# Hitenze/Preconditioned_Additive_Gaussian_Processes_with_Fourier_Acceleration

Hardware: AMD Instinct MI355X
Metric: kernel matvecs/sec + PCG wall-time to 1e-6, n=1e6 d=32 additive, 1/2/4/8 GPU (higher is better)
Workload: dtype f64; 1 GPU; additive NFFT matvec, n=1000000, d=32, 32 x 1-D windows, Gaussian f=1 l=1 mu=0.01 (BASELINE configs[2]); n=1000000, d=32, nwindows=32, parallelism=single

## Files before the change

preconditioned_additive_gaussian_processes_with_fourier_acceleration_amd/csrc/internal.h:

```cpp
#pragma once

#include <hip/hip_runtime.h>

#include <cstdint>
#include <cstdio>
#include <memory>
#include <utility>
#include <string>
#include <vector>

#include "../../include/nfft4gp_amd.h"

namespace nfft4gp_amd {

constexpr int kNos = 64;
constexpr int kBand = 32;
constexpr int kM = 4;
constexpr int kTaps = 2 * kM + 2;
constexpr int kDeg = 7;
constexpr int kNC = kDeg + 1;
constexpr int kR = 16;
constexpr int kWave = 64;
constexpr int kPad = 32;
constexpr int kMaxBlock = 4096 - kPad;
// ... 77 lines not shown
struct AdditivePlan;
int build_layout_dev(const uint32_t* d_qc, int n, int nw, int B, int CG, AdditivePlan& P, hipStream_t s, int rec = 5);

struct DevLayout {
   uint16_t* meta = nullptr;
   uint32_t* lo = nullptr;
   uint32_t* q = nullptr;
   int* tile_off = nullptr;
   int* cmax = nullptr;
   long long ntiles = 0;
   size_t bytes = 0;
};

constexpr int kMdMaxDim = 5;
constexpr int kMdTiledMaxDim = 3;
struct MdComp {
   int d = 0;
   int hicount = 1;
   long long u_off = 0;
};
struct MdPlan {
   bool on = false;
   bool gfix_per_window = false;
   int maxd = 1;
   long long G = 0;
   long long Cmax = 0;
   long long M = 0;
   std::vector<MdComp> comps;
   MdComp* d_comps = nullptr;
   int* d_u = nullptr;
   double* d_psi = nullptr;
   double* d_grid = nullptr;
   double2* d_F[2] = {nullptr, nullptr};
   double2* d_Mo[2] = {nullptr, nullptr};
   double2* d_B[4] = {nullptr, nullptr, nullptr, nullptr};
   double* d_h[2] = {nullptr, nullptr};
   double* d_bh = nullptr;
   double* d_bhd = nullptr;
   double* d_dot_part = nullptr;
   unsigned int* d_dot_ticket = nullptr;
   int* d_perm = nullptr;
   int4* d_items = nullptr;
   int nitems = 0;
   bool lines = false;
   double* d_part = nullptr;
   unsigned long long* d_gfix = nullptr;
   unsigned long long* d_xmax = nullptr;
   double psi_max = 0.0;
};

struct AdditivePlan {
   int n_global = 0, row_begin = 0, row_end = 0, n = 0;
   int nw = 0, dw = 0, skip_last = 0;
   std::vector<int> comp_dims;
   int d = 0;
   std::vector<int> comp_feature;
   bool points_ready = false;
   std::vector<double> comp_scale;
   std::vector<double> comp_centre;
   std::vector<double> comp_sigma;
   int kernel = 0;
   double f = 1.0, l = 1.0, mu = 0.0;
   double weight = 1.0;
   double diag = 1.0;
   int B = kMaxBlock, CG = 3, ngroups = 0, nblocks = 0;
   int rec = 5;
   int spread_variant = -1;
   int spread_fold = 1;
   bool det = false;
   double* d_hb = nullptr;
   int nparts = 0;
   DevLayout dl;
   double* d_part = nullptr;
   double* d_w = nullptr;
   double* d_wd = nullptr;
   double* d_H = nullptr;
   double* d_Hd = nullptr;
   double* d_C = nullptr;
   double* d_dot_part = nullptr;
   unsigned int* d_dot_ticket = nullptr;
   double* d_part2 = nullptr;
   double* d_gsum = nullptr;
   int fused_grid = -1;
   bool cells33 = false;
   double* d_hsum = nullptr;
   int hsum_par = 0;
   double* d_H2 = nullptr;
   double* d_xs = nullptr;
   double* d_ys = nullptr;
   MdPlan md;
   bool timing = false;
   hipEvent_t* kev = nullptr;
   double ms[3] = {0, 0, 0};
   long long cnt[3] = {0, 0, 0};
};

int upload_tap_coeffs();
int launch_spread(const AdditivePlan& P, const double* d_x, double* d_part, hipStream_t stream);
int launch_grid(const AdditivePlan& P, const double* d_part, int nparts, int grad, hipStream_t stream);
int launch_spread_grid(AdditivePlan& P, const double* d_x, int grad, hipStream_t stream);
int launch_grid_from_sum(const AdditivePlan& P, const double* d_gridsum, int grad, hipStream_t stream);
constexpr int kPeerInline = 8;
struct PeerArgs {
   char* const* bufs = nullptr;
   char* inl[kPeerInline] = {};
   char* own = nullptr;
   int world = 0;
   unsigned int epoch = 0;
   unsigned int* err = nullptr;
   long long slot_doubles = 0;
   long long spin = 0;
};
int launch_reduce_parts(const AdditivePlan& P, const double* d_part, double* d_gridsum, hipStream_t stream,
                        const PeerArgs* A = nullptr);
int launch_shard_finish_split(const AdditivePlan& P, const double* d_gridsum, double alpha, const double* d_x,
                              double beta, double* d_y, int S, hipStream_t stream, const PeerArgs* A = nullptr,
                              const double* d_part = nullptr);
int launch_peer_grid(const AdditivePlan& P, const PeerArgs& A, const double* d_part, hipStream_t stream);
int launch_peer_sum(const AdditivePlan& P, const PeerArgs& A, double* d_grid, hipStream_t stream);
int launch_interp(const AdditivePlan& P, int grad, double alpha, const double* d_x, double beta, double* d_y,
                  hipStream_t stream, double* d_dot = nullptr);
int launch_interp_blocks(const AdditivePlan& P, double alpha, const double* d_x, double beta, double* d_y, int b0,
                         int b1, hipStream_t stream);
int launch_matvec2(AdditivePlan& P, double alpha, const double* x0, const double* x1, double beta, double* y0,
                   double* y1, hipStream_t stream);
int pick_spread_variant(const AdditivePlan& P);
bool grid_atomic(const AdditivePlan& P);
int pick_interp_threads(const AdditivePlan& P);
bool pick_interp_hl(const AdditivePlan& P);
int pick_hl_slots(const AdditivePlan& P);
int pick_interp2_threads();
bool pick_fused_grid(const AdditivePlan& P);
int launch_matvec_fused(AdditivePlan& P, double alpha, const double* d_x, double beta, double* d_y, hipStream_t stream,
                        double* d_dot = nullptr);
int additive_matvec_multi(void* str, int nv, double alpha, const double* const* X, double beta, double* const* Y);
int additive_matvec_dot(void* str, const double* d_x, double* d_y, double* d_dot);
AdditivePlan* additive_plan_of(void* str);
bool additive_fused_dot_ok(void* str);

struct NysDev {
   int n = 0, k = 0;
   double eta = 0.0;
   double* U = nullptr;
   float* Uf = nullptr;
   double* s = nullptr;
   double* w = nullptr;
   double* part = nullptr;
   int nblk = 0;
   double setup_ms[4] = {0.0, 0.0, 0.0, 0.0};
   std::vector<double> hs;
   bool grad = false;
   double f2 = 0.0;
   double *Kall = nullptr, *dU = nullptr, *G = nullptr, *Gt = nullptr, *GdKG = nullptr, *D = nullptr;
   double *vk = nullptr, *vn = nullptr;
};
void nys_free(NysDev* N);
constexpr int kNysRows = 2048;
int nys_alloc_scratch(NysDev* N);
int gemm_f64(bool transA, int M, int N, int K, const double* A, long long lda, const double* B, long long ldb,
             double* C, long long ldc, hipStream_t s);
int sym_eig_host(const std::vector<double>& A, int n, std::vector<double>& w, std::vector<double>& V);
int chol_inverse_host(std::vector<double>& A, int k);
int lu_solve_host(std::vector<double>& A, int n, std::vector<double>& B, int nrhs, double* logabsdet = nullptr,
                  int* sign = nullptr, std::vector<int>* piv_out = nullptr);
void lu_subst_host(const std::vector<double>& A, int n, const std::vector<int>& piv, std::vector<double>& B, int nrhs);
int lu_solve_dev(double* A, int n, double* B, int nrhs, hipStream_t s, double* logabsdet = nullptr,
// ... 161 lines not shown
```

preconditioned_additive_gaussian_processes_with_fourier_acceleration_amd/csrc/nfft_api.cpp:

```cpp
#include <dlfcn.h>
#include <hip/hip_runtime.h>

#include <array>
#include <algorithm>
#include <atomic>
#include <chrono>
#include <thread>
#include <cmath>
#include <cstdio>
#include <cstdlib>
#include <cstring>
#include <mutex>
#include <vector>

#include "internal.h"
#include "reduce.hpp"

using namespace nfft4gp_amd;

namespace nfft4gp_amd {

namespace {
std::recursive_mutex g_rand_mu;
int g_rand_depth = 0;
// ... 416 lines not shown
   if (!dy) {
      yd = P.d_ys;
      if (beta != 0.0) NFFT4GP_HIP_CHECK(hipMemcpyAsync(yd, y, sizeof(double) * ny, hipMemcpyHostToDevice, s));
   }
   if (plan_apply_dev(E, grad, alpha, xd, beta, yd)) return -1;
   if (!dy) NFFT4GP_HIP_CHECK(hipMemcpyAsync(y, yd, sizeof(double) * ny, hipMemcpyDeviceToHost, s));
   NFFT4GP_HIP_CHECK(hipStreamSynchronize(s));
   return 0;
}

PlanExt* additive_plan(void* str)
{
   if (!str) return nullptr;
   return (PlanExt*)((nfft4gp_kernel*)str)->_external;
}


int omp_threads_in_process()
{
   using fn_t = int (*)();
   static fn_t f = (fn_t)dlsym(RTLD_DEFAULT, "omp_get_max_threads");
   return f ? std::max(1, f()) : 1;
}

nfft4gp_kernel* kernel_struct_create(int max_n, int omp = 0)
{
   nfft4gp_kernel* k = (nfft4gp_kernel*)calloc(1, sizeof(nfft4gp_kernel));
   k->_max_n = max_n;
   k->_omp = omp;
   k->_ldwork = (size_t)max_n * (size_t)(omp ? omp_threads_in_process() : 1);
   k->_dwork = (double*)malloc(sizeof(double) * std::max<size_t>(1, k->_ldwork));
   return k;
}

int setup_common(void* str, int kernel, int n, int ldim, double** Kp, double** dKp)
{
   if (Kp == NULL || dKp == NULL) {
      printf("Error: NFFT kernel requires Kp and dKp to be not NULL.\n");
      return -1;
   }
   nfft4gp_kernel* kd = (nfft4gp_kernel*)str;
   PlanExt* E = additive_plan(str);
   if (!E) return -1;
   (void)n;
   (void)ldim;
   if (plan_setup(E->P, kd->_buffer, kernel, kd->_params[0], kd->_params[1], kd->_noise_level)) return -1;
   *Kp = (double*)str;
   *dKp = (double*)str;
   return 0;
}

int default_block(int n)
{
   if (n >= 200 * kMaxBlock) return kMaxBlock;
   if (n >= 40 * 2032) return 2032;
   return 1024;
}

void env_layout(AdditivePlan& P)
{
   P.B = default_block(P.n);
   {
      const int nw = std::max(P.nw, 1), nblocks = std::max(1, (P.n + P.B - 1) / P.B);
      auto pick = [&](int cgmax) {
         const int ngroups = (nw + cgmax - 1) / cgmax;
         P.CG = (nw + ngroups - 1) / ngroups;
         return ngroups;
      };
      if ((long long)pick(4) * nblocks < 384) pick(3);
   }
   if (const char* e = getenv("NFFT4GP_AMD_BLOCK")) {
      const int v = atoi(e);
      if (v >= 256) P.B = std::min(v, kMaxBlock) & ~15;
   }
   if (const char* e = getenv("NFFT4GP_AMD_CG")) {
      const int v = atoi(e);
      if (v >= 1 && v <= 64) P.CG = v;
   }
   if (const char* e = getenv("NFFT4GP_AMD_SPREAD_VARIANT")) P.spread_variant = atoi(e);
   if (const char* e = getenv("NFFT4GP_AMD_SPREAD_FOLD")) P.spread_fold = atoi(e) != 0;
   if (const char* e = getenv("NFFT4GP_AMD_DET")) P.det = atoi(e) != 0;
   if (const char* e = getenv("NFFT4GP_AMD_PRECISION")) P.rec = atoi(e) == 32 ? 4 : 5;
   if (const char* e = getenv("NFFT4GP_AMD_FUSED_GRID")) P.fused_grid = atoi(e) != 0;
}

void* additive_create(double* data, int n_global, int ldim, int d, int* windows, int nwindows, int dwindows, int rb,
                      int re)
{
   nfft4gp_kernel* kd = kernel_struct_create(3 * n_global);
   kd->_iparams[0] = nwindows;
   kd->_iparams[1] = dwindows;
   int skip_window = 1;
   kd->_iparams[2] = 0;
   while (skip_window < dwindows && windows[nwindows * dwindows - skip_window] < 0) {
      skip_window++;
      kd->_iparams[2]++;
   }
   kd->_ibufferp = (int**)malloc(sizeof(int*));
   kd->_ibufferp[0] = windows;
   kd->_buffer = (double*)malloc(sizeof(double) * (size_t)n_global * nwindows * dwindows);
   kd->_own_buffer = 1;
   PlanExt* E = new PlanExt();
   AdditivePlan& P = E->P;
   P.n_global = n_global;
   P.row_begin = rb;
   P.row_end = re;
   P.n = re - rb;
   P.nw = nwindows;
   P.dw = dwindows;
   P.d = d;
   P.skip_last = kd->_iparams[2];
   P.weight = 1.0 / (double)nwindows;
   env_layout(P);
   double* dst = kd->_buffer;
   const int* fw = windows;
   for (int i = 0; i < nwindows; i++) {
      int actual = 0;
      for (int j = 0; j < dwindows; j++) {
         if (fw[0] >= 0) {
            memcpy(dst, data + (size_t)fw[0] * ldim, sizeof(double) * n_global);
            if (actual == 0) P.comp_feature.push_back(fw[0]);
            fw++;
            dst += n_global;
            actual++;
         }
      }
      if (actual == 0) P.comp_feature.push_back(-1);
      P.comp_dims.push_back(actual);
   }
   kd->_external = E;
   return kd;
}

}

namespace nfft4gp_amd {
bool additive_fused_dot_ok(void* str)
{
   PlanExt* E = additive_plan(str);
   if (!E || !E->P.points_ready) return false;
   const AdditivePlan& P = E->P;
   if (P.row_begin != 0 || P.row_end != P.n_global) return false;
   return P.md.on || P.nblocks <= kRedMaxBlocks;
}

int additive_matvec_dot(void* str, const double* d_x, double* d_y, double* d_dot)
{
   PlanExt* E = additive_plan(str);
   if (!E || !E->P.points_ready) return -1;
   AdditivePlan& P = E->P;
   hipStream_t s = current_stream();
   if (P.md.on) {
      if (md_spread(P, d_x, P.md.d_grid, s) || md_grid(P, P.md.d_grid, 0, s)) return -1;
      return md_interp(P, 0, 1.0, d_x, 0.0, d_y, s, d_dot);
   }
   if (use_fused(P, s)) return launch_matvec_fused(P, 1.0, d_x, 0.0, d_y, s, d_dot);
   if (launch_spread_grid(P, d_x, 0, s)) return -1;
   return launch_interp(P, 0, 1.0, d_x, 0.0, d_y, s, d_dot);
}
}

namespace nfft4gp_amd {
int additive_matvec_multi(void* str, int nv, double alpha, const double* const* X, double beta, double* const* Y)
{
   PlanExt* E = additive_plan(str);
   if (!E || !E->P.points_ready) return -1;
// ... 662 lines not shown
```

preconditioned_additive_gaussian_processes_with_fourier_acceleration_amd/csrc/nfft_kernels.hip:

```cpp
#include <hip/hip_ext.h>
#include <hip/hip_runtime.h>

#include <algorithm>
#include <cmath>
#include <cstdio>
#include <vector>

#include "internal.h"
#include "reduce.hpp"

namespace nfft4gp_amd {

constexpr int kGridThreads = 1024;
constexpr int kMomStride = kNC + 1;
constexpr int kMomWin = kNC * kNos + 4;
template <int MOMT>
__host__ __device__ constexpr int mom_doubles_per_window()
{
   return MOMT ? kMomWin : kNos * kMomStride;
}
template <int MOMT>
__device__ __forceinline__ int mom_index(int cl, int cell, int d)
{
   return MOMT ? cl * kMomWin + d * kNos + cell : (cl * kNos + cell) * kMomStride + d;
// ... 96 lines not shown
   const int per = (nloc + nwaves - 1) / nwaves;
   const uint32_t* hw = reinterpret_cast<const uint32_t*>(s_alpha);
   uint32_t m = 0;
   for (int e = wave * per + lane; e < min(nloc, (wave + 1) * per); e += 64) m = max(m, hw[2 * e + 1] & 0x7FFFFFFFu);
   for (int off = 32; off > 0; off >>= 1) m = max(m, (uint32_t)__shfl_xor((int)m, off, 64));
   if (lane == 0) {
      s_red[wave] = m;
      __hip_atomic_fetch_add(s_red + nwaves, 1u, __ATOMIC_RELEASE, __HIP_MEMORY_SCOPE_WORKGROUP);
   }
}
template <int THREADS>
__device__ __forceinline__ uint32_t det_max_wait(uint32_t* s_red)
{
   constexpr int nwaves = THREADS / 64;
   while (__hip_atomic_load(s_red + nwaves, __ATOMIC_ACQUIRE, __HIP_MEMORY_SCOPE_WORKGROUP) < (uint32_t)nwaves)
      __builtin_amdgcn_s_sleep(1);
   uint32_t m = 0;
#pragma unroll
   for (int w = 0; w < nwaves; w++) m = max(m, s_red[w]);
   return (uint32_t)__builtin_amdgcn_readfirstlane((int)m) >> 20;
}

__device__ __forceinline__ uint32_t det_interp_exp(const double* __restrict__ hb, int nw)
{
   double Y = 0.0;
   for (int c = 0; c < nw; c++) Y += hb[c];
   const uint32_t bY = ((uint32_t)__double2hiint(Y) >> 20) & 0x7FFu;
   return min(bY + 2u, 2046u);
}

template <int REC>
__device__ __forceinline__ int tile_at(TileRegs& cur, const uint16_t* __restrict__ meta,
                                       const uint32_t* __restrict__ lo, const uint32_t* __restrict__ qarr, int t, int t1)
{
   if (t < t1) load_tile<REC>(cur, meta, lo, qarr, t, threadIdx.x & 63);
   return t;
}

__device__ __forceinline__ void gather_h(double (&h)[kNC], const double* __restrict__ H, uint32_t mt)
{
   const double2* src = reinterpret_cast<const double2*>(H + (size_t)mt * kNC);
#pragma unroll
   for (int d = 0; d < kNC; d += 2) {
      const double2 v = src[d / 2];
      h[d] = v.x;
      h[d + 1] = v.y;
   }
}
__device__ __forceinline__ void gather_h_lds(double (&h)[kNC], const double* row, int stride)
{
#pragma unroll
   for (int d = 0; d < kNC; d++) h[d] = row[d * stride];
}

template <int REC, bool DET>
__device__ __forceinline__ void interp_run(const TileRegs& cur, const double (&h)[kNC], double C)
{
#pragma unroll
   for (int r = 0; r < kR; r++) {
      const uint32_t off = slot_off<REC>(cur, r);
      const double u = q_to_s(cur.qq[r]);
      double v = h[kNC - 1];
#pragma unroll
      for (int d = kNC - 2; d >= 0; d--) v = fma(v, u, h[d]);
      lds_add(off, DET ? det_round(v, C) : v);
   }
}

constexpr int kEpMax = 8;

template <int THREADS>
__device__ __forceinline__ void ep_prefetch(double (&xe)[kEpMax], double (&ye)[kEpMax], const double* __restrict__ x,
                                            const double* __restrict__ y, int base, int nloc, double beta)
{
   static_assert(kMaxBlock <= kEpMax * THREADS, "a block's epilogue values fit the threads' registers");
#pragma unroll
   for (int k = 0; k < kEpMax; k++) {
      const int j = threadIdx.x + k * THREADS;
      xe[k] = (j < nloc) ? x[(size_t)base + j] : 0.0;
      ye[k] = (beta != 0.0 && j < nloc) ? y[(size_t)base + j] : 0.0;
   }
}

template <int THREADS, bool DOT>
__device__ __forceinline__ double ep_plain(const double (&xe)[kEpMax], const double (&ye)[kEpMax], const double* s_y,
                                           double* __restrict__ y, int base, int nloc, double alpha, double beta,
                                           double f, double mu)
{
   const double ff = f * f;
   double dacc = 0.0;
#pragma unroll
   for (int k = 0; k < kEpMax; k++) {
      const int j = threadIdx.x + k * THREADS;
      if (j >= nloc) break;
      const double v = ff * (s_y[j] + mu * xe[k]);
      const double yo = (beta == 0.0) ? alpha * v : fma(beta, ye[k], alpha * v);
      y[(size_t)base + j] = yo;
      if (DOT) dacc = fma(yo, xe[k], dacc);
   }
   return dacc;
}

template <int THREADS>
__device__ __forceinline__ void ep_dot_finish(double dacc, double* s_scr, double* __restrict__ dot_part,
                                              unsigned int* __restrict__ dot_ticket, double* __restrict__ dot_out)
{
   dacc = block_sum0_s<THREADS>(dacc, s_scr);
   double tot;
   if (grid_total_s<THREADS>(dacc, dot_part, dot_ticket, &tot, reinterpret_cast<int*>(s_scr + 2 * (THREADS / 64)),
                             s_scr + THREADS / 64) &&
       threadIdx.x == 0)
      *dot_out = tot;
}

constexpr bool kFoldMfmaOk = kNC == 8 && kTaps <= 12 && kNos == 64;
template <int REC>
__device__ __forceinline__ void fold_tap_operand(double (&a)[2], int lane)
{
   const int i = lane & 15, k = lane >> 4;
   const double* ct = REC == 4 ? c_taps_u : c_taps;
#pragma unroll
   for (int ks = 0; ks < 2; ks++) a[ks] = i < kTaps ? ct[i * kNC + 4 * ks + k] : 0.0;
}
__device__ __forceinline__ double fold_window_mfma(const double (&a)[2], double* mrow, double* grow89, int lane)
{
   typedef double f64x4 __attribute__((ext_vector_type(4)));
   const int i = lane & 15, k = lane >> 4;
   double bm[2][4];
#pragma unroll
   for (int ks = 0; ks < 2; ks++)
#pragma unroll
      for (int cb = 0; cb < 4; cb++) bm[ks][cb] = mrow[(4 * ks + k) * kNos + 16 * cb + i];
#pragma unroll
   for (int cb = 0; cb < 4; cb++) {
      f64x4 acc = {0.0, 0.0, 0.0, 0.0};
      acc = __builtin_amdgcn_mfma_f64_16x16x4f64(a[0], bm[0][cb], acc, 0, 0, 0);
      acc = __builtin_amdgcn_mfma_f64_16x16x4f64(a[1], bm[1][cb], acc, 0, 0, 0);
      mrow[k * kNos + 16 * cb + i] = acc[0];
      mrow[(4 + k) * kNos + 16 * cb + i] = acc[1];
      if (k < kTaps - 8) grow89[k * kNos + 16 * cb + i] = acc[2];
   }
   __builtin_amdgcn_fence(__ATOMIC_RELEASE, "wavefront");
   __builtin_amdgcn_wave_barrier();
   __builtin_amdgcn_fence(__ATOMIC_ACQUIRE, "wavefront");
   double v = 0.0;
#pragma unroll
   for (int tp = 0; tp < kTaps; tp++) {
      const int cell = (lane + kM - tp) & (kNos - 1);
      v += tp < 8 ? mrow[tp * kNos + cell] : grow89[(tp - 8) * kNos + cell];
   }
   return v;
}

constexpr int kFgCells = 33;
constexpr int kFgSpan = kFgCells + kTaps - 1;
constexpr int kFgSpan0 = (kNos - 16 - kM) & (kNos - 1);

template <int THREADS, bool TIMELINE = false, int MOMT = 1, bool DET = false, int REC = 5, bool PIPE = false>
__global__ __launch_bounds__(THREADS, 6) void k_spread(const uint16_t* __restrict__ meta,
                                                      const uint32_t* __restrict__ lo,
                                                      const uint32_t* __restrict__ qarr,
                                                      const int* __restrict__ tile_off, const int* __restrict__ cmax,
                                                      const double* __restrict__ x, int n, int B, int nblocks,
                                                      int ngroups, int CG, int nw, double* __restrict__ part,
                                                      double* __restrict__ gsum, int fold)
{
   extern __shared__ __attribute__((aligned(16))) double smem[];
   const int Bp = B + kPad;
   double* s_alpha = smem;
   double* s_mom = smem + Bp;
   uint32_t* s_red = reinterpret_cast<uint32_t*>(s_mom + CG * mom_doubles_per_window<MOMT>());

   const int xcd = blockIdx.x & 7;
   const int rest = blockIdx.x >> 3;
   const int g = rest % ngroups;
   const int b = (rest / ngroups) * 8 + xcd;
   if (b >= nblocks) return;
   if (TIMELINE) stamp(0);

   const int tid = threadIdx.x;
// ... 563 lines not shown
   }
}

template <int THREADS, bool DET = false, int REC = 5>
__global__ __launch_bounds__(THREADS) void k_interp_hl(const uint16_t* __restrict__ meta, const uint32_t* __restrict__ lo,
                                                       const uint32_t* __restrict__ qarr, const int* __restrict__ tile_off,
                                                       const double* __restrict__ H, const double* __restrict__ x,
                                                       double* __restrict__ y, int n, int B, int ngroups, int CG, int nw,
                                                       double alpha, double beta, double f, double mu,
                                                       const double* __restrict__ hb, int ns)
{
   extern __shared__ __attribute__((aligned(16))) double smem[];
   const int Bp = B + kPad;
   double* s_y = smem;
   double* s_H = smem + Bp;
   int* s_ready = reinterpret_cast<int*>(s_H + (size_t)ns * CG * kHlWin);
   int* s_done = s_ready + ns;
   int* s_toff = s_done + ngroups;
   const int b = blockIdx.x;
   const int tid = threadIdx.x;
   const int base = b * B;
   const int nloc = min(B, n - base);
   const int lane = tid & 63;
   const int wave = tid >> 6;
   constexpr int nwaves = THREADS / 64;
   const int gbase = b * ngroups;
   TileRegs cur;
   const int t1 = tile_off[gbase + ngroups];
   int t = tile_at<REC>(cur, meta, lo, qarr, tile_off[gbase] + wave, t1);
   double xe[kEpMax], ye[kEpMax];
   ep_prefetch<THREADS>(xe, ye, x, y, base, nloc, beta);
   for (int i = tid; i < Bp; i += THREADS) s_y[i] = 0.0;
   for (int i = tid; i < ngroups; i += THREADS) s_done[i] = 0;
   for (int i = tid; i <= ngroups; i += THREADS) s_toff[i] = tile_off[gbase + i];
   if (tid < ns) s_ready[tid] = tid;
   if (wave < ns && wave < ngroups) hl_stage_wave(s_H, H, wave, wave, CG, nw, lane);
   const double Cy = DET ? det_grid(det_interp_exp(hb, nw)) : 0.0;
   __syncthreads();

   int g = 0, gslot = 0;
   int gend = s_toff[1];
   auto leave = [&](int gl) {
      int old = 0;
      if (lane == 0) old = __hip_atomic_fetch_add(s_done + gl, 1, __ATOMIC_ACQ_REL, __HIP_MEMORY_SCOPE_WORKGROUP);
      old = __builtin_amdgcn_readfirstlane(old);
      if (old == nwaves - 1 && gl + ns < ngroups) {
         const int sl = gl % ns;
         hl_stage_wave(s_H, H, gl + ns, sl, CG, nw, lane);
         __builtin_amdgcn_fence(__ATOMIC_RELEASE, "workgroup");
         if (lane == 0) __hip_atomic_store(s_ready + sl, gl + ns, __ATOMIC_RELEASE, __HIP_MEMORY_SCOPE_WORKGROUP);
      }
   };
   for (; t < t1; t = tile_at<REC>(cur, meta, lo, qarr, t + nwaves, t1)) {
      while (t >= gend) {
         leave(g);
         g++;
         gend = s_toff[g + 1];
         gslot = g % ns;
         if (g >= ns) {
            for (long spin = 0; spin < (1l << 24); spin++) {
               if (__hip_atomic_load(s_ready + gslot, __ATOMIC_ACQUIRE, __HIP_MEMORY_SCOPE_WORKGROUP) == g) break;
               __builtin_amdgcn_s_sleep(1);
            }
         }
      }
      const int cl = (int)(cur.mt >> 6) - g * CG;
      const int cell = (int)(cur.mt & 63u);
      double h[kNC];
      gather_h_lds(h, s_H + ((size_t)gslot * CG + cl) * kHlWin + cell, kNos);
      interp_run<REC, DET>(cur, h, Cy);
   }
   for (; g < ngroups; g++) leave(g);
   __syncthreads();

   ep_plain<THREADS, false>(xe, ye, s_y, y, base, nloc, alpha, beta, f, mu);
}

constexpr int kFgWin = kNC * kFgCells + 1;
constexpr int kFgRow = kNos + 1;
constexpr int kFgQuads = (kFgSpan + 3) / 4;
constexpr int kFgHs = 4 * kFgQuads + 1;
constexpr int kFgLdsWin = kFgWin + kFgHs + 2 * kFgRow;

template <int THREADS, bool DOT = false, int REC = 5>
__global__ __launch_bounds__(THREADS) void k_interp_fg(
    const uint16_t* __restrict__ meta, const uint32_t* __restrict__ lo, const uint32_t* __restrict__ qarr,
    const int* __restrict__ tile_off, const double* __restrict__ gsum, double* __restrict__ gclear,
    const double* __restrict__ wcirc, const double* __restrict__ x, double* __restrict__ y, int n, int B, int ngroups,
    double alpha, double beta, double f, double mu, double* __restrict__ dot_part,
    unsigned int* __restrict__ dot_ticket, double* __restrict__ dot_out, int nw)
{
   static_assert(THREADS % (4 * kNC) == 0 && kNC == 8, "a thread keeps its degree and cell quarter over the build");
   static_assert(kFgSpan % 6 == 0, "the circulant's steps go six per trip");
   extern __shared__ __attribute__((aligned(16))) double smem[];
   const int Bp = B + kPad;
   double* s_y = smem;
   double* s_H = smem + Bp;
   double* s_h = s_H + (size_t)nw * kFgWin;
   double* s_g = s_h + (size_t)nw * kFgHs;
   double* s_w = s_g + (size_t)nw * kFgRow;
   double* s_scr = s_w + (size_t)nw * kFgRow;
   const int b = blockIdx.x;
   const int tid = threadIdx.x;
   const int base = b * B;
   const int nloc = min(B, n - base);
   TileRegs cur;
   const int t1 = tile_off[(b + 1) * ngroups];
   int t = tile_at<REC>(cur, meta, lo, qarr, tile_off[b * ngroups] + (tid >> 6), t1);
   double ct[kTaps];
#pragma unroll
   for (int tp = 0; tp < kTaps; tp++) ct[tp] = c_taps[tp * kNC + (tid & (kNC - 1))];
   for (int i = tid; i < nw * kNos; i += THREADS) {
      const int o = (i >> 6) * kFgRow + (i & (kNos - 1));
      s_g[o] = gsum[i];
      s_w[o] = wcirc[i];
   }
   if (b == 0)
      for (int i = tid; i < nw * kNos; i += THREADS) gclear[i] = 0.0;
   for (int i = tid; i < Bp; i += THREADS) s_y[i] = 0.0;
   __syncthreads();
   for (int it = tid; it < nw * kFgQuads; it += THREADS) {
      const int w = it / kFgQuads, k0 = 4 * (it % kFgQuads);
      const double* gw = s_g + w * kFgRow;
      const double* ww = s_w + w * kFgRow;
      double r3 = ww[(k0 + 3) & (kNos - 1)], r2 = ww[(k0 + 2) & (kNos - 1)], r1 = ww[(k0 + 1) & (kNos - 1)], r0 = ww[k0];
      double a0 = 0.0, a1 = 0.0, a2 = 0.0, a3 = 0.0;
#pragma unroll 6
      for (int j = 0; j < kFgSpan; j++) {
         const double gj = gw[(kFgSpan0 + j) & (kNos - 1)];
         a0 = fma(r0, gj, a0);
         a1 = fma(r1, gj, a1);
         a2 = fma(r2, gj, a2);
         a3 = fma(r3, gj, a3);
         r3 = r2, r2 = r1, r1 = r0;
         r0 = ww[(k0 - j - 1) & (kNos - 1)];
      }
      double* hw = s_h + w * kFgHs + k0;
      hw[0] = a0, hw[1] = a1, hw[2] = a2, hw[3] = a3;
   }
   __syncthreads();
   {
      const int d = tid & (kNC - 1), seg = (tid >> 3) & 3;
      const int c0 = seg ? 8 * seg + 1 : 0, c1 = 8 * seg + 9;
      for (int w = tid >> 5; w < nw; w += THREADS / 32) {
         const double* hw = s_h + w * kFgHs + c0;
         double hv[kTaps + 8];
#pragma unroll
         for (int j = 0; j < kTaps + 8; j++) hv[j] = hw[j];
         double acc[9];
#pragma unroll
         for (int k = 0; k < 9; k++) acc[k] = 0.0;
#pragma unroll
         for (int tp = 0; tp < kTaps; tp++) {
#pragma unroll
            for (int k = 0; k < 9; k++) acc[k] = fma(hv[k + tp], ct[tp], acc[k]);
         }
         double* dst = s_H + (size_t)w * kFgWin + d * kFgCells + c0;
#pragma unroll
         for (int k = 0; k < 9; k++)
            if (c0 + k < c1) dst[k] = acc[k];
      }
   }
   __syncthreads();
   double xe[kEpMax], ye[kEpMax];
   ep_prefetch<THREADS>(xe, ye, x, y, base, nloc, beta);

   for (; t < t1; t = tile_at<REC>(cur, meta, lo, qarr, t + THREADS / 64, t1)) {
      const int ci = min((int)((cur.mt + 16u) & 63u), kFgCells - 1);
      double h[kNC];
      gather_h_lds(h, s_H + (size_t)(cur.mt >> 6) * kFgWin + ci, kFgCells);
      interp_run<REC, false>(cur, h, 0.0);
   }
   __syncthreads();

   const double dacc = ep_plain<THREADS, DOT>(xe, ye, s_y, y, base, nloc, alpha, beta, f, mu);
   if (DOT) ep_dot_finish<THREADS>(dacc, s_scr, dot_part, dot_ticket, dot_out);
}


template <int THREADS, bool DET = false, int REC = 5>
__global__ __launch_bounds__(THREADS) void k_interp2(const uint16_t* __restrict__ meta,
                                                     const uint32_t* __restrict__ lo,
                                                     const uint32_t* __restrict__ qarr,
                                                     const int* __restrict__ tile_off, const double* __restrict__ H,
                                                     size_t h_rs, const double* __restrict__ x0,
                                                     const double* __restrict__ x1, double* __restrict__ y0,
                                                     double* __restrict__ y1, int n, int B, int ngroups, double alpha,
                                                     double beta, double f, double mu, const double* __restrict__ hb,
                                                     int nw)
{
   extern __shared__ __attribute__((aligned(16))) double smem[];
   const int Bp = B + kPad;
   double* s_y0 = smem;
   double* s_y1 = smem + Bp;
   const int b = blockIdx.x;
   const int tid = threadIdx.x;
   const int base = b * B;
   const int nloc = min(B, n - base);
   const int lane = tid & 63;
   const int wave = tid >> 6;
   constexpr int nwaves = THREADS / 64;
   const int t0 = tile_off[b * ngroups];
   const int t1 = tile_off[(b + 1) * ngroups];
   TileRegs cur;
   int t = tile_at<REC>(cur, meta, lo, qarr, t0 + wave, t1);
   for (int i = tid; i < Bp; i += THREADS) s_y0[i] = s_y1[i] = 0.0;
   double C0 = 0.0, C1 = 0.0;
   if (DET) {
      C0 = det_grid(det_interp_exp(hb, nw));
      C1 = det_grid(det_interp_exp(hb + 2 * nw, nw));
   }
   __syncthreads();
   const double* H1 = H + h_rs;
   for (; t < t1; t += nwaves) {
      const size_t hoff = (size_t)cur.mt * kNC;
      double h0[kNC], h1[kNC];
#pragma unroll
      for (int d = 0; d < kNC; d += 2) {
         const double2 v0 = *reinterpret_cast<const double2*>(H + hoff + d);
         const double2 v1 = *reinterpret_cast<const double2*>(H1 + hoff + d);
         h0[d] = v0.x;
         h0[d + 1] = v0.y;
         h1[d] = v1.x;
         h1[d + 1] = v1.y;
      }
#pragma unroll
      for (int r = 0; r < kR; r++) {
         const uint32_t off = slot_off<REC>(cur, r);
         const double u = q_to_s(cur.qq[r]);
         double v0 = h0[kNC - 1], v1 = h1[kNC - 1];
#pragma unroll
         for (int d = kNC - 2; d >= 0; d--) {
            v0 = fma(v0, u, h0[d]);
            v1 = fma(v1, u, h1[d]);
         }
         lds_add(off, DET ? det_round(v0, C0) : v0);
         lds_add(off + 8u * (uint32_t)Bp, DET ? det_round(v1, C1) : v1);
      }
      if (t + nwaves < t1) load_tile<REC>(cur, meta, lo, qarr, t + nwaves, lane);
   }
   __syncthreads();
   const double ff = f * f;
   for (int j = tid; j < nloc; j += THREADS) {
      const size_t gj = (size_t)base + j;
      const double v0 = ff * (s_y0[j] + mu * x0[gj]);
      const double v1 = ff * (s_y1[j] + mu * x1[gj]);
      y0[gj] = (beta == 0.0) ? alpha * v0 : fma(beta, y0[gj], alpha * v0);
      y1[gj] = (beta == 0.0) ? alpha * v1 : fma(beta, y1[gj], alpha * v1);
   }
}

template <typename F, typename... A>
static void launch_ev(F fn, dim3 grid, dim3 block, size_t lds, hipStream_t s, const hipEvent_t* ev, A... args)
{
   if (ev)
      hipExtLaunchKernelGGL(fn, grid, block, (std::uint32_t)lds, s, ev[0], ev[1], 0u, args...);
   else
      hipLaunchKernelGGL(fn, grid, block, lds, s, args...);
// ... 14 lines not shown
   return sizeof(double) * ((size_t)P.B + kPad) * (grad ? 2 : 1) + kRedScratch;
}

int upload_tap_coeffs()
{
   static bool done[64] = {false};
   int dev = 0;
   NFFT4GP_HIP_CHECK(hipGetDevice(&dev));
   if (dev < 0 || dev >= 64) return -1;
   if (!done[dev]) {
      NFFT4GP_HIP_CHECK(hipMemcpyToSymbol(HIP_SYMBOL(c_taps_u), tap_poly_coeffs().data(), sizeof(double) * kTaps * kNC));
      std::vector<double> C = tap_poly_coeffs();
      for (int t = 0; t < kTaps; t++)
         for (int d = 0; d < kNC; d++) C[t * kNC + d] = std::ldexp(C[t * kNC + d], -32 * d);
      NFFT4GP_HIP_CHECK(hipMemcpyToSymbol(HIP_SYMBOL(c_taps), C.data(), sizeof(double) * kTaps * kNC));
      done[dev] = true;
   }
   return 0;
}

typedef void (*SpreadFn)(const uint16_t*, const uint32_t*, const uint32_t*, const int*, const int*, const double*, int,
                         int, int, int, int, int, double*, double*, int);
constexpr int kSpreadThreads = 512;
static const SpreadFn kSpreadFns[2][2][4] = {
    {{k_spread<kSpreadThreads>, k_spread<kSpreadThreads, true>, k_spread<kSpreadThreads, false, 0>,
      k_spread<kSpreadThreads, false, 1, false, 5, true>},
     {k_spread<kSpreadThreads, false, 1, true>, k_spread<kSpreadThreads, true, 1, true>,
      k_spread<kSpreadThreads, false, 0, true>, k_spread<kSpreadThreads, false, 1, true, 5, true>}},
    {{k_spread<kSpreadThreads, false, 1, false, 4>, k_spread<kSpreadThreads, true, 1, false, 4>,
      k_spread<kSpreadThreads, false, 0, false, 4>, k_spread<kSpreadThreads, false, 1, false, 4, true>},
     {k_spread<kSpreadThreads, false, 1, true, 4>, k_spread<kSpreadThreads, true, 1, true, 4>,
      k_spread<kSpreadThreads, false, 0, true, 4>, k_spread<kSpreadThreads, false, 1, true, 4, true>}}};
constexpr int kNumSpreadVariants = 4;
constexpr size_t kInfinityCacheBytes = 256ull << 20;
int pick_spread_variant(const AdditivePlan& P)
{
   int v = P.spread_variant;
   if (v < 0) v = P.dl.bytes > kInfinityCacheBytes ? 3 : 0;
   return std::min(v, kNumSpreadVariants - 1);
}
static SpreadFn spread_fn(const AdditivePlan& P)
{
   return kSpreadFns[P.rec == 4 ? 1 : 0][P.det ? 1 : 0][pick_spread_variant(P)];
}

constexpr int kInterpThreads = 1024;
typedef void (*InterpFn)(const uint16_t*, const uint32_t*, const uint32_t*, const int*, const double*,
                         const double*, const double*, double*, int, int, int, double, double, double, double,
                         double, double*, unsigned int*, double*, const double*, int);

template <int T, int REC>
static InterpFn interp_fn_t(bool grad, bool dot, bool det)
{
   if (grad) return det ? k_interp<true, T, false, true, REC> : k_interp<true, T, false, false, REC>;
   if (dot) return det ? k_interp<false, T, true, true, REC> : k_interp<false, T, true, false, REC>;
   return det ? k_interp<false, T, false, true, REC> : k_interp<false, T, false, false, REC>;
}
static InterpFn interp_fn(bool grad, bool dot, bool small, bool det, int rec)
{
   if (rec == 4) return small ? interp_fn_t<512, 4>(grad, dot, det) : interp_fn_t<kInterpThreads, 4>(grad, dot, det);
   return small ? interp_fn_t<512, 5>(grad, dot, det) : interp_fn_t<kInterpThreads, 5>(grad, dot, det);
}
constexpr int kInterp2Threads = 1024;
typedef void (*Interp2Fn)(const uint16_t*, const uint32_t*, const uint32_t*, const int*, const double*, size_t,
                          const double*, const double*, double*, double*, int, int, int, double, double, double, double,
                          const double*, int);
template <int REC>
static Interp2Fn interp2_fn_t(bool det, bool small)
{
   if (small) return det ? k_interp2<512, true, REC> : k_interp2<512, false, REC>;
   return det ? k_interp2<kInterp2Threads, true, REC> : k_interp2<kInterp2Threads, false, REC>;
}
static Interp2Fn interp2_fn(bool det, bool small, int rec)
{
   return rec == 4 ? interp2_fn_t<4>(det, small) : interp2_fn_t<5>(det, small);
}
typedef void (*InterpPartFn)(const uint16_t*, const uint32_t*, const uint32_t*, const int*, const double*, double*, int,
                             int, int, int, double);
static InterpPartFn interp_part_fn(int rec) { return rec == 4 ? k_interp_part<512, 4> : k_interp_part<512, 5>; }

typedef void (*InterpFgFn)(const uint16_t*, const uint32_t*, const uint32_t*, const int*, const double*, double*,
                           const double*, const double*, double*, int, int, int, double, double, double, double,
                           double*, unsigned int*, double*, int);
static InterpFgFn interp_fg_fn(bool dot, int rec)
{
   if (rec == 4) return dot ? k_interp_fg<kInterpThreads, true, 4> : k_interp_fg<kInterpThreads, false, 4>;
   return dot ? k_interp_fg<kInterpThreads, true, 5> : k_interp_fg<kInterpThreads, false, 5>;
}

typedef void (*InterpHlFn)(const uint16_t*, const uint32_t*, const uint32_t*, const int*, const double*, const double*,
                           double*, int, int, int, int, int, double, double, double, double, const double*, int);
static InterpHlFn interp_hl_fn(bool small, bool det, int rec)
{
   if (rec == 4)
      return small ? (det ? k_interp_hl<512, true, 4> : k_interp_hl<512, false, 4>)
                   : (det ? k_interp_hl<1024, true, 4> : k_interp_hl<1024, false, 4>);
   return small ? (det ? k_interp_hl<512, true, 5> : k_interp_hl<512, false, 5>)
                : (det ? k_interp_hl<1024, true, 5> : k_interp_hl<1024, false, 5>);
}
bool pick_interp_hl(const AdditivePlan& P)
{
   static const int v = getenv("NFFT4GP_AMD_INTERP_HL") ? atoi(getenv("NFFT4GP_AMD_INTERP_HL")) : -1;
   return (v < 0 ? P.dl.bytes > kInfinityCacheBytes : v != 0) && P.ngroups >= 1;
}
int pick_interp_threads(const AdditivePlan& P)
{
   static const int forced = getenv("NFFT4GP_AMD_INTERP_THREADS") ? atoi(getenv("NFFT4GP_AMD_INTERP_THREADS")) : 0;
   return forced == 512 || (forced != 1024 && P.nblocks >= 512) ? 512 : kInterpThreads;
}
int pick_hl_slots(const AdditivePlan& P)
{
   static const int slots_env = getenv("NFFT4GP_AMD_HL_SLOTS") ? atoi(getenv("NFFT4GP_AMD_HL_SLOTS")) : 0;
   int ns = std::max(2, std::min(slots_env > 0 ? slots_env : 2, pick_interp_threads(P) == 512 ? 2 : 6));
   while (ns > 2 && hl_lds_bytes(P.B, P.CG, P.ngroups, ns) > kMaxDynamicLds) ns--;
   return ns;
}
int pick_interp2_threads()
{
   static const int forced = getenv("NFFT4GP_AMD_INTERP2_THREADS") ? atoi(getenv("NFFT4GP_AMD_INTERP2_THREADS")) : 0;
   return forced == 512 ? 512 : kInterp2Threads;
}

static std::vector<const void*> interp_kernels()
{
   std::vector<const void*> v;
   for (int sm = 0; sm < 2; sm++)
      for (int det = 0; det < 2; det++)
         for (int rec = 4; rec <= 5; rec++) v.push_back((const void*)interp_hl_fn(sm, det, rec));
   for (int g = 0; g < 2; g++)
      for (int d = 0; d < 2; d++)
         for (int sm = 0; sm < 2; sm++)
            for (int det = 0; det < 2; det++)
               for (int rec = 4; rec <= 5; rec++) v.push_back((const void*)interp_fn(g, d && !g, sm, det, rec));
   for (int det = 0; det < 2; det++)
      for (int sm = 0; sm < 2; sm++)
         for (int rec = 4; rec <= 5; rec++) v.push_back((const void*)interp2_fn(det, sm, rec));
   for (int rec = 4; rec <= 5; rec++) v.push_back((const void*)interp_part_fn(rec));
   for (int d = 0; d < 2; d++)
      for (int rec = 4; rec <= 5; rec++) v.push_back((const void*)interp_fg_fn(d, rec));
   return v;
}
static std::vector<const void*> spread_kernels()
{
   std::vector<const void*> v;
   for (const auto& byrec : kSpreadFns)
      for (const auto& bydet : byrec)
         for (const SpreadFn f : bydet) v.push_back((const void*)f);
   return v;
}

static bool lds_ready()
{
   static const bool ok = [] {
      std::vector<const void*> v = interp_kernels();
      for (const void* f : spread_kernels()) v.push_back(f);
      for (const void* f : v)
         (void)hipFuncSetAttribute(f, hipFuncAttributeMaxDynamicSharedMemorySize, (int)kMaxDynamicLds);
      (void)hipGetLastError();
      hipFuncAttributes a;
      for (const void* f : v)
         if (hipFuncGetAttributes(&a, f) != hipSuccess || a.sharedSizeBytes != 0) return false;
      return true;
   }();
   if (!ok) fprintf(stderr, "nfft4gp_amd: a matvec kernel has static LDS; its absolute LDS addressing would be wrong\n");
   return ok;
}

static int launch_spread_to(const AdditivePlan& P, const double* d_x, double* d_part, double* d_gsum,
                            hipStream_t stream)
{
   if (P.dl.ntiles == 0 || P.n == 0) return 0;
   if (!lds_ready()) return -1;
   const SpreadFn fn = spread_fn(P);
   const int gridx = ((P.nblocks + 7) / 8) * 8 * P.ngroups;
   launch_ev(fn, dim3(gridx), dim3(kSpreadThreads), spread_lds_bytes(P), stream, P.kev ? P.kev + 0 : nullptr,
             P.dl.meta, P.dl.lo, P.dl.q, P.dl.tile_off, (const int*)P.dl.cmax, d_x, P.n, P.B, P.nblocks, P.ngroups,
             P.CG, P.nw, d_part, d_gsum, P.spread_fold);
   NFFT4GP_HIP_CHECK(hipGetLastError());
   return 0;
}

int launch_spread(const AdditivePlan& P, const double* d_x, double* d_part, hipStream_t stream)
{
   return launch_spread_to(P, d_x, d_part, nullptr, stream);
}

constexpr int kAtomicGridMaxBlocks = 512;
bool grid_atomic(const AdditivePlan& P)
{
   static const int v = getenv("NFFT4GP_AMD_GRID_ATOMIC") ? atoi(getenv("NFFT4GP_AMD_GRID_ATOMIC")) : -1;
   if (P.det || v == 0) return false;
   return v > 0 || P.nblocks <= kAtomicGridMaxBlocks;
}

static int launch_k_grid(const AdditivePlan& P, const double* src, int nparts, int from_sum, int grad, int clear_sum,
                         hipStream_t stream, double* H2 = nullptr, size_t part_rs = 0, size_t h_rs = 0)
{
   launch_ev(k_grid, dim3(P.nw, H2 ? 2 : 1), dim3(kGridThreads), 0, stream, P.kev && !H2 ? P.kev + 2 : nullptr, src,
             nparts, (const double*)P.d_w, (const double*)P.d_wd, H2 ? H2 : P.d_H, P.d_Hd, grad, from_sum,
             (long long)part_rs, (long long)h_rs, P.det ? P.d_hb : (double*)nullptr, clear_sum);
   NFFT4GP_HIP_CHECK(hipGetLastError());
   return 0;
}

int launch_spread_grid(AdditivePlan& P, const double* d_x, int grad, hipStream_t stream)
{
   if (!grid_atomic(P) || P.nblocks == 0) {
      if (launch_spread(P, d_x, P.d_part, stream)) return -1;
      return launch_grid(P, P.d_part, P.nparts, grad, stream);
   }
   if (!P.d_gsum) {
      NFFT4GP_HIP_CHECK(hipMalloc((void**)&P.d_gsum, sizeof(double) * (size_t)P.nw * kNos));
      NFFT4GP_HIP_CHECK(hipMemsetAsync(P.d_gsum, 0, sizeof(double) * (size_t)P.nw * kNos, stream));
   }
   if (launch_spread_to(P, d_x, nullptr, P.d_gsum, stream)) return -1;
   return launch_k_grid(P, P.d_gsum, 1, 1, grad, 1, stream);
}

int launch_grid(const AdditivePlan& P, const double* d_part, int nparts, int grad, hipStream_t stream)
{
   return launch_k_grid(P, d_part, nparts, 0, grad, 0, stream);
}
// ... 28 lines not shown
   if (A.slot_doubles != (long long)P.nw * kNos) return -1;
   hipLaunchKernelGGL(k_grid_sum_yinit, dim3(P.nw), dim3(kGridThreads), 0, stream, (const double*)nullptr,
                      (const double*)P.d_w, P.d_H, (double*)nullptr, (const double*)nullptr, 0, 0.0, 0.0, A,
                      P.nblocks ? d_part : (const double*)P.d_w, P.nblocks ? P.nparts : 0);
   NFFT4GP_HIP_CHECK(hipGetLastError());
   return 0;
}

int launch_reduce_parts(const AdditivePlan& P, const double* d_part, double* d_gridsum, hipStream_t stream,
                        const PeerArgs* A)
{
   PeerArgs a = A ? *A : PeerArgs{};
   if (A && A->slot_doubles != (long long)P.nw * kNos) return -1;
   hipLaunchKernelGGL(k_reduce_parts, dim3(P.nw), dim3(kGridThreads), 0, stream, d_part, P.nblocks ? P.nparts : 0,
                      P.nw, d_gridsum, a);
   NFFT4GP_HIP_CHECK(hipGetLastError());
   return 0;
}

int launch_peer_sum(const AdditivePlan& P, const PeerArgs& A, double* d_grid, hipStream_t stream)
{
   if (A.slot_doubles != (long long)P.nw * kNos) return -1;
   hipLaunchKernelGGL(k_peer_sum, dim3(P.nw), dim3(kGridThreads), 0, stream, A, d_grid);
   NFFT4GP_HIP_CHECK(hipGetLastError());
   return 0;
}

int launch_interp(const AdditivePlan& P, int grad, double alpha, const double* d_x, double beta, double* d_y,
                  hipStream_t stream, double* d_dot)
{
   if (P.n == 0) return 0;
   if (!lds_ready()) return -1;
   if (d_dot && (grad || P.nblocks > kRedMaxBlocks)) {
      fprintf(stderr, "nfft4gp_amd: fused matvec-dot needs a plain matvec and <= %d blocks\n", kRedMaxBlocks);
      return -1;
   }
   const bool small = pick_interp_threads(P) == 512;
   if (!grad && !d_dot && pick_interp_hl(P)) {
      const int ns = pick_hl_slots(P);
      launch_ev(interp_hl_fn(small, P.det, P.rec), dim3(P.nblocks), dim3(small ? 512 : kInterpThreads),
                hl_lds_bytes(P.B, P.CG, P.ngroups, ns), stream, P.kev ? P.kev + 4 : nullptr, P.dl.meta, P.dl.lo,
                P.dl.q, P.dl.tile_off, (const double*)P.d_H, d_x, d_y, P.n, P.B, P.ngroups, P.CG, P.nw, alpha, beta,
                P.f, P.mu * P.diag, (const double*)P.d_hb, ns);
      NFFT4GP_HIP_CHECK(hipGetLastError());
      return 0;
   }
   const InterpFn fn = interp_fn(grad, d_dot != nullptr, small, P.det, P.rec);
   launch_ev(fn, dim3(P.nblocks), dim3(small ? 512 : kInterpThreads), interp_lds_bytes(P, grad), stream,
             P.kev ? P.kev + 4 : nullptr, P.dl.meta, P.dl.lo, P.dl.q, P.dl.tile_off, (const double*)P.d_H,
             (const double*)P.d_Hd, d_x, d_y, P.n, P.B, P.ngroups, alpha, beta, P.f, P.mu * P.diag, P.diag,
             P.d_dot_part, P.d_dot_ticket, d_dot, (const double*)P.d_hb, P.nw);
   NFFT4GP_HIP_CHECK(hipGetLastError());
   return 0;
}

static size_t fg_lds_bytes(int B, int nw)
{
   return sizeof(double) * ((size_t)B + kPad) + sizeof(double) * (size_t)nw * kFgLdsWin + kRedScratch;
}
constexpr int kFusedMaxBlocks = 256;
bool pick_fused_grid(const AdditivePlan& P)
{
   if (P.fused_grid == 0 || !P.cells33 || P.md.on || P.det || P.nblocks == 0 || P.n == 0) return false;
   if (P.row_begin != 0 || P.row_end != P.n_global) return false;
   if (!grid_atomic(P) || pick_interp_threads(P) != kInterpThreads || pick_interp_hl(P)) return false;
   if (fg_lds_bytes(P.B, P.nw) > kMaxDynamicLds) return false;
   return P.fused_grid > 0 || P.nblocks <= kFusedMaxBlocks;
}

int launch_matvec_fused(AdditivePlan& P, double alpha, const double* d_x, double beta, double* d_y, hipStream_t stream,
                        double* d_dot)
{
   if (!lds_ready()) return -1;
   if (d_dot && P.nblocks > kRedMaxBlocks) return -1;
   const size_t ns = (size_t)P.nw * kNos;
   if (!P.d_hsum) {
      NFFT4GP_HIP_CHECK(hipMalloc((void**)&P.d_hsum, sizeof(double) * 2 * ns));
      NFFT4GP_HIP_CHECK(hipMemsetAsync(P.d_hsum, 0, sizeof(double) * 2 * ns, stream));
      P.hsum_par = 0;
   }
   double* S = P.d_hsum + (size_t)P.hsum_par * ns;
   double* Sother = P.d_hsum + (size_t)(1 - P.hsum_par) * ns;
   if (launch_spread_to(P, d_x, nullptr, S, stream)) return -1;
   launch_ev(interp_fg_fn(d_dot != nullptr, P.rec), dim3(P.nblocks), dim3(kInterpThreads), fg_lds_bytes(P.B, P.nw),
             stream, P.kev ? P.kev + 4 : nullptr, P.dl.meta, P.dl.lo, P.dl.q, P.dl.tile_off, (const double*)S, Sother,
             (const double*)P.d_w, d_x, d_y, P.n, P.B, P.ngroups, alpha, beta, P.f, P.mu * P.diag, P.d_dot_part,
             P.d_dot_ticket, d_dot, P.nw);
   NFFT4GP_HIP_CHECK(hipGetLastError());
   P.hsum_par ^= 1;
   return 0;
}

int launch_interp_blocks(const AdditivePlan& P, double alpha, const double* d_x, double beta, double* d_y, int b0,
                         int b1, hipStream_t stream)
{
   if (P.n == 0 || b1 <= b0) return 0;
   if (!lds_ready()) return -1;
   const size_t off = (size_t)b0 * P.B;
   hipLaunchKernelGGL(interp_fn(false, false, false, P.det, P.rec), dim3(b1 - b0), dim3(kInterpThreads),
                      interp_lds_bytes(P, 0), stream, P.dl.meta, P.dl.lo, P.dl.q, P.dl.tile_off + (size_t)b0 * P.ngroups,
                      (const double*)P.d_H, (const double*)P.d_Hd, d_x + off, d_y + off, P.n - (int)off, P.B, P.ngroups,
                      alpha, beta, P.f, P.mu * P.diag, P.diag, (double*)nullptr, (unsigned int*)nullptr,
                      (double*)nullptr, (const double*)P.d_hb, P.nw);
   NFFT4GP_HIP_CHECK(hipGetLastError());
   return 0;
}

int launch_matvec2(AdditivePlan& P, double alpha, const double* x0, const double* x1, double beta, double* y0,
                   double* y1, hipStream_t stream)
{
   if (P.n == 0) return 0;
   if (P.md.on) return -1;
   if (!lds_ready()) return -1;
   const size_t part_rs = (size_t)std::max(1, P.nparts) * P.nw * kNos;
   const size_t h_rs = (size_t)P.nw * kNos * kNC;
   if (!P.d_part2) NFFT4GP_HIP_CHECK(hipMalloc((void**)&P.d_part2, sizeof(double) * 2 * part_rs));
   if (!P.d_H2) NFFT4GP_HIP_CHECK(hipMalloc((void**)&P.d_H2, sizeof(double) * 2 * h_rs));
   if (launch_spread(P, x0, P.d_part2, stream) || launch_spread(P, x1, P.d_part2 + part_rs, stream)) return -1;
   if (launch_k_grid(P, P.d_part2, P.nparts, 0, 0, 0, stream, P.d_H2, part_rs, h_rs)) return -1;
   const size_t lds_i = sizeof(double) * 2 * ((size_t)P.B + kPad);
   const bool small = pick_interp2_threads() == 512;
   hipLaunchKernelGGL(interp2_fn(P.det, small, P.rec), dim3(P.nblocks), dim3(small ? 512 : kInterp2Threads), lds_i, stream,
                      P.dl.meta, P.dl.lo,
                      P.dl.q, P.dl.tile_off, (const double*)P.d_H2, h_rs, x0, x1, y0, y1, P.n, P.B, P.ngroups, alpha,
                      beta, P.f, P.mu * P.diag, (const double*)P.d_hb, P.nw);
   NFFT4GP_HIP_CHECK(hipGetLastError());
   return 0;
}

}
```

Baseline: 14850 matvecs/s.

## Overlap fused-interp prologue loads with tile prefetch and use nontemporal output stores

The fused grid+interp kernel now issues the first grid-sum/weight loads into registers and loads the first two tiles before and during the LDS setup and H computation. This hides the global-load latency of the prologue behind other work. Output stores in the epilogue become nontemporal to avoid polluting cache. An optional timeline variant with timestamp stamps is added behind an env var. The extra live registers may reduce occupancy.

```diff
diff --git a/preconditioned_additive_gaussian_processes_with_fourier_acceleration_amd/csrc/internal.h b/preconditioned_additive_gaussian_processes_with_fourier_acceleration_amd/csrc/internal.h
--- a/preconditioned_additive_gaussian_processes_with_fourier_acceleration_amd/csrc/internal.h
+++ b/preconditioned_additive_gaussian_processes_with_fourier_acceleration_amd/csrc/internal.h
@@ -183,6 +183,7 @@
    double* d_part2 = nullptr;
    double* d_gsum = nullptr;
    int fused_grid = -1;
+   int interp_timeline = 0;
    bool cells33 = false;
    double* d_hsum = nullptr;
    int hsum_par = 0;
diff --git a/preconditioned_additive_gaussian_processes_with_fourier_acceleration_amd/csrc/nfft_api.cpp b/preconditioned_additive_gaussian_processes_with_fourier_acceleration_amd/csrc/nfft_api.cpp
--- a/preconditioned_additive_gaussian_processes_with_fourier_acceleration_amd/csrc/nfft_api.cpp
+++ b/preconditioned_additive_gaussian_processes_with_fourier_acceleration_amd/csrc/nfft_api.cpp
@@ -522,6 +522,7 @@
    if (const char* e = getenv("NFFT4GP_AMD_DET")) P.det = atoi(e) != 0;
    if (const char* e = getenv("NFFT4GP_AMD_PRECISION")) P.rec = atoi(e) == 32 ? 4 : 5;
    if (const char* e = getenv("NFFT4GP_AMD_FUSED_GRID")) P.fused_grid = atoi(e) != 0;
+   if (const char* e = getenv("NFFT4GP_AMD_INTERP_TIMELINE")) P.interp_timeline = atoi(e) != 0;
 }
 
 void* additive_create(double* data, int n_global, int ldim, int d, int* windows, int nwindows, int dwindows, int rb,
diff --git a/preconditioned_additive_gaussian_processes_with_fourier_acceleration_amd/csrc/nfft_kernels.hip b/preconditioned_additive_gaussian_processes_with_fourier_acceleration_amd/csrc/nfft_kernels.hip
--- a/preconditioned_additive_gaussian_processes_with_fourier_acceleration_amd/csrc/nfft_kernels.hip
+++ b/preconditioned_additive_gaussian_processes_with_fourier_acceleration_amd/csrc/nfft_kernels.hip
@@ -202,7 +202,7 @@
    }
 }
 
-template <int THREADS, bool DOT>
+template <int THREADS, bool DOT, bool NT = false>
 __device__ __forceinline__ double ep_plain(const double (&xe)[kEpMax], const double (&ye)[kEpMax], const double* s_y,
                                            double* __restrict__ y, int base, int nloc, double alpha, double beta,
                                            double f, double mu)
@@ -215,7 +215,10 @@
       if (j >= nloc) break;
       const double v = ff * (s_y[j] + mu * xe[k]);
       const double yo = (beta == 0.0) ? alpha * v : fma(beta, ye[k], alpha * v);
-      y[(size_t)base + j] = yo;
+      if (NT)
+         __builtin_nontemporal_store(yo, y + (size_t)base + j);
+      else
+         y[(size_t)base + j] = yo;
       if (DOT) dacc = fma(yo, xe[k], dacc);
    }
    return dacc;
@@ -945,7 +948,7 @@
 constexpr int kFgHs = 4 * kFgQuads + 1;
 constexpr int kFgLdsWin = kFgWin + kFgHs + 2 * kFgRow;
 
-template <int THREADS, bool DOT = false, int REC = 5>
+template <int THREADS, bool DOT = false, int REC = 5, bool TIMELINE = false>
 __global__ __launch_bounds__(THREADS) void k_interp_fg(
     const uint16_t* __restrict__ meta, const uint32_t* __restrict__ lo, const uint32_t* __restrict__ qarr,
     const int* __restrict__ tile_off, const double* __restrict__ gsum, double* __restrict__ gclear,
@@ -967,21 +970,45 @@
    const int tid = threadIdx.x;
    const int base = b * B;
    const int nloc = min(B, n - base);
-   TileRegs cur;
+   constexpr int nwaves = THREADS / 64;
+   if (TIMELINE) stamp(0);
    const int t1 = tile_off[(b + 1) * ngroups];
-   int t = tile_at<REC>(cur, meta, lo, qarr, tile_off[b * ngroups] + (tid >> 6), t1);
+   int t = tile_off[b * ngroups] + (tid >> 6);
+   constexpr int kFgRegTrips = 2;
+   const int ns = nw * kNos;
+   double gv[kFgRegTrips], wv[kFgRegTrips];
+#pragma unroll
+   for (int k = 0; k < kFgRegTrips; k++) {
+      const int i = min(tid + k * THREADS, ns - 1);
+      gv[k] = gsum[i];
+      wv[k] = wcirc[i];
+   }
    double ct[kTaps];
 #pragma unroll
    for (int tp = 0; tp < kTaps; tp++) ct[tp] = c_taps[tp * kNC + (tid & (kNC - 1))];
-   for (int i = tid; i < nw * kNos; i += THREADS) {
+   for (int i = tid + kFgRegTrips * THREADS; i < ns; i += THREADS) {
       const int o = (i >> 6) * kFgRow + (i & (kNos - 1));
       s_g[o] = gsum[i];
       s_w[o] = wcirc[i];
    }
+   TileRegs cur, nxt;
+   __builtin_amdgcn_sched_barrier(0);
+   load_tile<REC>(cur, meta, lo, qarr, max(min(t, t1 - 1), 0), tid & 63);
+   __builtin_amdgcn_sched_barrier(0);
+   for (int i = tid; i < Bp; i += THREADS) s_y[i] = 0.0;
+#pragma unroll
+   for (int k = 0; k < kFgRegTrips; k++) {
+      const int i = tid + k * THREADS;
+      if (i < ns) {
+         const int o = (i >> 6) * kFgRow + (i & (kNos - 1));
+         s_g[o] = gv[k];
+         s_w[o] = wv[k];
+      }
+   }
    if (b == 0)
-      for (int i = tid; i < nw * kNos; i += THREADS) gclear[i] = 0.0;
-   for (int i = tid; i < Bp; i += THREADS) s_y[i] = 0.0;
-   __syncthreads();
+      for (int i = tid; i < ns; i += THREADS) gclear[i] = 0.0;
+   __syncthreads();
+   if (TIMELINE) stamp(1);
    for (int it = tid; it < nw * kFgQuads; it += THREADS) {
       const int w = it / kFgQuads, k0 = 4 * (it % kFgQuads);
       const double* gw = s_g + w * kFgRow;
@@ -1001,6 +1028,7 @@
       double* hw = s_h + w * kFgHs + k0;
       hw[0] = a0, hw[1] = a1, hw[2] = a2, hw[3] = a3;
    }
+   load_tile<REC>(nxt, meta, lo, qarr, max(min(t + nwaves, t1 - 1), 0), tid & 63);
    __syncthreads();
    {
       const int d = tid & (kNC - 1), seg = (tid >> 3) & 3;
@@ -1025,18 +1053,30 @@
       }
    }
    __syncthreads();
+   if (TIMELINE) stamp(2);
    double xe[kEpMax], ye[kEpMax];
    ep_prefetch<THREADS>(xe, ye, x, y, base, nloc, beta);
 
-   for (; t < t1; t = tile_at<REC>(cur, meta, lo, qarr, t + THREADS / 64, t1)) {
-      const int ci = min((int)((cur.mt + 16u) & 63u), kFgCells - 1);
+   auto run = [&](const TileRegs& T) {
+      const int ci = min((int)((T.mt + 16u) & 63u), kFgCells - 1);
       double h[kNC];
-      gather_h_lds(h, s_H + (size_t)(cur.mt >> 6) * kFgWin + ci, kFgCells);
-      interp_run<REC, false>(cur, h, 0.0);
-   }
-   __syncthreads();
-
-   const double dacc = ep_plain<THREADS, DOT>(xe, ye, s_y, y, base, nloc, alpha, beta, f, mu);
+      gather_h_lds(h, s_H + (size_t)(T.mt >> 6) * kFgWin + ci, kFgCells);
+      interp_run<REC, false>(T, h, 0.0);
+   };
+   if (t < t1) {
+      run(cur);
+      const int tn = t + nwaves;
+      t = t1;
+      if (tn < t1) {
+         t = tile_at<REC>(cur, meta, lo, qarr, tn + nwaves, t1);
+         run(nxt);
+      }
+   }
+   for (; t < t1; t = tile_at<REC>(cur, meta, lo, qarr, t + nwaves, t1)) run(cur);
+   __syncthreads();
+   if (TIMELINE) stamp(3);
+
+   const double dacc = ep_plain<THREADS, DOT, true>(xe, ye, s_y, y, base, nloc, alpha, beta, f, mu);
    if (DOT) ep_dot_finish<THREADS>(dacc, s_scr, dot_part, dot_ticket, dot_out);
 }
 
@@ -1217,8 +1257,10 @@
 typedef void (*InterpFgFn)(const uint16_t*, const uint32_t*, const uint32_t*, const int*, const double*, double*,
                            const double*, const double*, double*, int, int, int, double, double, double, double,
                            double*, unsigned int*, double*, int);
-static InterpFgFn interp_fg_fn(bool dot, int rec)
-{
+static InterpFgFn interp_fg_fn(bool dot, int rec, bool tl)
+{
+   if (tl && !dot)
+      return rec == 4 ? k_interp_fg<kInterpThreads, false, 4, true> : k_interp_fg<kInterpThreads, false, 5, true>;
    if (rec == 4) return dot ? k_interp_fg<kInterpThreads, true, 4> : k_interp_fg<kInterpThreads, false, 4>;
    return dot ? k_interp_fg<kInterpThreads, true, 5> : k_interp_fg<kInterpThreads, false, 5>;
 }
@@ -1272,7 +1314,8 @@
          for (int rec = 4; rec <= 5; rec++) v.push_back((const void*)interp2_fn(det, sm, rec));
    for (int rec = 4; rec <= 5; rec++) v.push_back((const void*)interp_part_fn(rec));
    for (int d = 0; d < 2; d++)
-      for (int rec = 4; rec <= 5; rec++) v.push_back((const void*)interp_fg_fn(d, rec));
+      for (int rec = 4; rec <= 5; rec++)
+         for (int tl = 0; tl < 2; tl++) v.push_back((const void*)interp_fg_fn(d, rec, tl));
    return v;
 }
 static std::vector<const void*> spread_kernels()
@@ -1467,8 +1510,8 @@
    double* S = P.d_hsum + (size_t)P.hsum_par * ns;
    double* Sother = P.d_hsum + (size_t)(1 - P.hsum_par) * ns;
    if (launch_spread_to(P, d_x, nullptr, S, stream)) return -1;
-   launch_ev(interp_fg_fn(d_dot != nullptr, P.rec), dim3(P.nblocks), dim3(kInterpThreads), fg_lds_bytes(P.B, P.nw),
-             stream, P.kev ? P.kev + 4 : nullptr, P.dl.meta, P.dl.lo, P.dl.q, P.dl.tile_off, (const double*)S, Sother,
+   launch_ev(interp_fg_fn(d_dot != nullptr, P.rec, P.interp_timeline != 0), dim3(P.nblocks), dim3(kInterpThreads),
+             fg_lds_bytes(P.B, P.nw), stream, P.kev ? P.kev + 4 : nullptr, P.dl.meta, P.dl.lo, P.dl.q, P.dl.tile_off, (const double*)S, Sother,
              (const double*)P.d_w, d_x, d_y, P.n, P.B, P.ngroups, alpha, beta, P.f, P.mu * P.diag, P.d_dot_part,
              P.d_dot_ticket, d_dot, P.nw);
    NFFT4GP_HIP_CHECK(hipGetLastError());
```

New measurement: 15380 matvecs/s (median of 6 runs). +3.6%, better.
